# jasonyaw/CDAE

Hardware: AMD Instinct MI355X
Metric: users/sec (whole node) K=200 ML-10M-shape; Recall@10 parity (higher is better)
Workload: dtype f32

## Files before the change

cdae_amd/binding.py:

```python
from __future__ import annotations

import contextlib
import ctypes as C
import os
from dataclasses import dataclass

import numpy as np

_HERE = os.path.dirname(os.path.abspath(__file__))
LIB_PATH = os.environ.get("CDAE_HIP_LIBRARY") or os.path.join(_HERE, "lib", "libcdae_hip.so")
DEV_LIB_PATH = os.path.join(os.path.dirname(_HERE), "build", "libcdae_hip_dev.so")

SQUARE, LOGISTIC, LOG, HINGE, SQUARED_HINGE, CROSS_ENTROPY, LOGM = range(7)

P_W, P_W_AG, P_V, P_V_AG, P_WU, P_WU_AG, P_B, P_B_AG, P_BP, P_BP_AG, P_UU, P_UU_AG = range(12)
P_UB, P_UB_AG = 12, 13
P_COUNT = 14

PLAN_FUSED_DECODE, PLAN_GEMM2_TN, PLAN_ROWS_FUSED = 1, 2, 4
IMF_DEFAULT_BATCH_USERS = 16
BPR_DEFAULT_BATCH_USERS = 8
NO_USER = 0xFFFFFFFF
DEFAULT_BATCH_USERS = 0

# ... 14 lines not shown
    _fields_ = [("wall_seconds", C.c_double), ("users", C.c_uint64), ("examples", C.c_uint64),
                ("batches", C.c_uint64), ("ms_sample", C.c_double), ("ms_sort", C.c_double),
                ("ms_encode", C.c_double), ("ms_decode", C.c_double), ("ms_hidden", C.c_double),
                ("ms_input", C.c_double), ("launches_decode", C.c_uint64)]

    def as_dict(self):
        return {n: getattr(self, n) for n, _ in self._fields_}


EXPORTS = {
    "cdae_hip_last_error": (C.c_char_p, []),
    "cdae_hip_abi_version": (C.c_int, []),
    "cdae_hip_create": (C.c_int, [C.POINTER(_Config), C.c_int, C.POINTER(C.c_void_p)]),
    "cdae_hip_create_mf": (C.c_int, [C.POINTER(_MfConfig), C.c_int, C.POINTER(C.c_void_p)]),
    "cdae_hip_destroy": (C.c_int, [C.c_void_p]),
    "cdae_hip_set_interactions": (C.c_int, [C.c_void_p, C.c_uint64, C.c_uint64, C.c_void_p, C.c_void_p]),
    "cdae_hip_row_stride": (C.c_uint32, [C.c_void_p]),
    "cdae_hip_default_batch_users": (C.c_uint32, [C.c_uint64]),
    "cdae_hip_mf_default_batch_users": (C.c_uint32, [C.c_uint64, C.c_uint32]),
    "cdae_hip_batch_users": (C.c_uint32, [C.c_void_p]),
    "cdae_hip_full_output_plan": (C.c_uint32, [C.c_void_p]),
    "cdae_hip_set_decode_fused": (C.c_int, [C.c_void_p, C.c_int]),
    "cdae_hip_decode_plan": (C.c_int, [C.c_void_p, C.POINTER(C.c_uint32), C.POINTER(C.c_uint32), C.POINTER(C.c_uint32)]),
    "cdae_hip_user_order": (C.c_int, [C.c_void_p, C.c_void_p, C.c_size_t]),
    "cdae_hip_set_user_id_offset": (C.c_int, [C.c_void_p, C.c_uint64]),
    "cdae_hip_init_params": (C.c_int, [C.c_void_p, C.c_uint64]),
    "cdae_hip_set_param": (C.c_int, [C.c_void_p, C.c_uint32, C.c_void_p, C.c_size_t]),
    "cdae_hip_get_param": (C.c_int, [C.c_void_p, C.c_uint32, C.c_void_p, C.c_size_t]),
    "cdae_hip_param_device_ptr": (C.c_int, [C.c_void_p, C.c_uint32, C.POINTER(C.c_void_p), C.POINTER(C.c_size_t)]),
    "cdae_hip_train_epoch": (C.c_int, [C.c_void_p, C.c_uint64, C.c_uint32, C.POINTER(Stats)]),
    "cdae_hip_train_users": (C.c_int, [C.c_void_p, C.c_uint64, C.c_uint32, C.c_uint64, C.c_uint64, C.POINTER(Stats)]),
    "cdae_hip_enqueue_users": (C.c_int, [C.c_void_p, C.c_uint64, C.c_uint32, C.c_uint64, C.c_uint64]),
    "cdae_hip_prefetch_users": (C.c_int, [C.c_void_p, C.c_uint64, C.c_uint32, C.c_uint64, C.c_uint64]),
    "cdae_hip_collect_stats": (C.c_int, [C.c_void_p, C.POINTER(Stats)]),
    "cdae_hip_train_one_user_corruption": (C.c_int, [C.c_void_p, C.c_uint64, C.c_void_p, C.c_size_t, C.c_void_p, C.c_size_t]),
    "cdae_hip_set_profiling": (C.c_int, [C.c_void_p, C.c_int]),
    "cdae_hip_set_profiling_families": (C.c_int, [C.c_void_p, C.c_uint32]),
    "cdae_hip_synchronize": (C.c_int, [C.c_void_p]),
    "cdae_hip_debug_sample_batch": (C.c_int, [C.c_void_p, C.c_uint64, C.c_uint32, C.c_uint64, C.c_uint32, C.c_uint32] + [C.c_void_p] * 8
                                    + [C.POINTER(C.c_uint64)]),
    "cdae_hip_encode": (C.c_int, [C.c_void_p, C.c_uint64, C.c_uint32, C.c_int, C.c_void_p, C.c_size_t, C.c_void_p]),
    "cdae_hip_data_loss": (C.c_int, [C.c_void_p, C.c_uint64, C.c_uint32, C.POINTER(C.c_double)]),
    "cdae_hip_penalty_loss": (C.c_int, [C.c_void_p, C.POINTER(C.c_double)]),
    "cdae_hip_recommend_all": (C.c_int, [C.c_void_p, C.c_uint64, C.c_uint64, C.c_uint32, C.c_void_p]),
    "cdae_hip_recommend_user": (C.c_int, [C.c_void_p, C.c_uint64, C.c_void_p, C.c_size_t, C.c_uint32, C.c_void_p]),
    "cdae_hip_recommend_rows": (C.c_int, [C.c_void_p, C.c_uint64, C.c_void_p, C.c_void_p, C.c_void_p, C.c_uint32, C.c_void_p, C.c_void_p]),
# ... 141 lines not shown
    def reset(self, train, seed: int = 0):
        self.set_interactions(train.num_users, train.num_items, train.train_ptr, train.train_col)
        self.init_params(seed)

    def init_params(self, seed: int):
        _chk(self.lib, self.lib.cdae_hip_init_params(self.h, seed))

    def user_order(self) -> np.ndarray:
        out = np.empty(self.num_users, dtype=np.uint32)
        _chk(self.lib, self.lib.cdae_hip_user_order(self.h, out.ctypes.data, out.size))
        return out

    @property
    def batch_users(self) -> int:
        return int(self.lib.cdae_hip_batch_users(self.h))

    def set_decode_fused(self, allow: bool):
        _chk(self.lib, self.lib.cdae_hip_set_decode_fused(self.h, int(bool(allow))))

    @property
    def decode_plan(self) -> dict:
        a, b, c = C.c_uint32(0), C.c_uint32(0), C.c_uint32(0)
        _chk(self.lib, self.lib.cdae_hip_decode_plan(self.h, C.byref(a), C.byref(b), C.byref(c)))
        return dict(hot_rows=int(a.value), late_rows=int(b.value), fused=bool(c.value))

    @property
    def full_output_plan(self) -> int:
        return int(self.lib.cdae_hip_full_output_plan(self.h))

    def _shape(self, which):
        K = self.cfg.num_dim
        if which in (P_BP, P_BP_AG):
            return (self.num_items,)
        if which in (P_B, P_B_AG):
            return (K,)
        if which in (P_WU, P_WU_AG, P_UU, P_UU_AG):
            return (self.num_users, K)
        return (self.num_items, K)

    def get(self, which) -> np.ndarray:
        out = np.empty(self._shape(which), dtype=np.float32)
        _chk(self.lib, self.lib.cdae_hip_get_param(self.h, which, out.ctypes.data, out.size))
        return out

    def set(self, which, arr):
        a = np.ascontiguousarray(arr, dtype=np.float32).reshape(self._shape(which))
        _chk(self.lib, self.lib.cdae_hip_set_param(self.h, which, a.ctypes.data, a.size))
# ... 361 lines not shown
```

cdae_amd/csrc/cdae_hip.hip:

```cpp
#include <hip/hip_runtime.h>

#include <cstring>

#include <rocprim/rocprim.hpp>

#include <algorithm>
#include <atomic>
#include <condition_variable>
#include <deque>
#include <mutex>
#include <thread>
#include <chrono>
#include <cmath>
#include <cstdarg>
#include <cstdlib>
#include <cstdio>
#include <cstring>
#include <numeric>
#include <string>
#include <vector>

#include "../../include/cdae_hip.h"
#include "cdae_internal.hpp"
#include "cdae_kernels.hpp"
// ... 60 lines not shown
  uint64_t U = 0, I = 0;
  uint32_t K = 0, Kp = 0, NI = 1, B = 0;
  uint64_t uid_offset = 0;
  cdae::HyperParams hp{};

  std::vector<int64_t> h_row_ptr;
  int64_t* d_row_ptr = nullptr;
  uint32_t* d_col = nullptr;
  uint32_t* d_item_order = nullptr;
  uint32_t hot_rows = 0;
  uint32_t late_rows = 0;
  float* d_Ghot = nullptr;
  uint32_t* d_hotdup = nullptr;
  uint32_t* d_late_bits = nullptr;
  uint32_t late_words = 0;
  bool fused_decode = false;
  bool fused_possible = false;
  bool allow_fused = true;
  uint32_t* h_err = nullptr;
  int err_slot = -1;
  uint32_t* d_fused_err = nullptr;
  cdae::FusedGeom fused_geo{};
  bool fused_geo_set = false;
  std::vector<float> h_rank_len;
  uint32_t* d_cold_map = nullptr;
  uint32_t num_cus = 256;
  cdae::DecodeLate decode_late() const { return cdae::DecodeLate{d_Ghot, d_hotdup, late_rows}; }
  cdae::LateFinish late_finish() { return cdae::LateFinish{d_Ghot, d_hotdup, d_item_order, d_D0, d_dup_corr, late_rows}; }
  bool full_unfused = false;
  std::vector<uint32_t> h_unit_ptr;
  uint32_t* d_rank_of = nullptr;
  uint32_t* d_unit_user = nullptr;
  uint32_t* d_unit_ptr = nullptr;
  uint32_t unit_cap = 0;
  float* d_Hpart = nullptr;
  uint32_t* d_uptr_tmp = nullptr;

  float* d_shared = nullptr;
  size_t n_shared = 0, n_matrix = 0;
  size_t off[CDAE_P_COUNT] = {0};
  size_t cnt[CDAE_P_COUNT] = {0};
  float* d_Wu = nullptr;
  float* d_Wu_ag = nullptr;
  float* d_Uu = nullptr;
  float* d_Uu_ag = nullptr;
  float* d_Ssum = nullptr;
// ... 394 lines not shown
    HIPCHK(rocprim::radix_sort_pairs(sort_tmp, h->sort_tmp_bytes, x.key16, x.sorted_key16, x.val, x.sorted_val,
                                     (size_t)bt.E, 0u, (unsigned)h->sort_bits, st));
    hipLaunchKernelGGL(segment_kernel<uint16_t>, seg_grid, dim3(256), 0, st, x.sorted_key16, x.sorted_val, (uint32_t)bt.E,
                       x.seg, x.seg + I, x.dup_count, h->dup_cap, x.dup_of_pos, x.dup_of_ex, h->dup_stripes,
                       (const uint32_t*)h->d_rank_of, x.seg + 2 * (size_t)I, x.seg + 3 * (size_t)I, shs ? I : 0xFFFFFFFFu);
  } else {
    HIPCHK(rocprim::radix_sort_pairs(sort_tmp, h->sort_tmp_bytes, x.item, x.sorted_item, x.val, x.sorted_val,
                                     (size_t)bt.E, 0u, (unsigned)h->sort_bits, st));
    hipLaunchKernelGGL(segment_kernel<uint32_t>, seg_grid, dim3(256), 0, st, x.sorted_item, x.sorted_val, (uint32_t)bt.E,
                       x.seg, x.seg + I, x.dup_count, h->dup_cap, x.dup_of_pos, x.dup_of_ex, h->dup_stripes,
                       (const uint32_t*)h->d_rank_of, x.seg + 2 * (size_t)I, x.seg + 3 * (size_t)I, shs ? I : 0xFFFFFFFFu);
  }
  CHK(pr.end());
  if (h->cfg.full_output && h->d_bits_train) {
    const uint32_t words = (I + 31) / 32;
    uint32_t* bits = h->d_bits_train + (size_t)b * h->bits_stride;
    hipLaunchKernelGGL(rated_bits_kernel, dim3((bt.nb + 3) / 4), dim3(256), 0, st, h->d_row_ptr, h->d_col, bt.s0, bt.nb, words, bits);
  }
  HIPCHK(hipEventRecord(x.ready, st));
  HIPCHK(hipGetLastError());
  return 0;
}

int fused_geometry(cdae_hip* h, uint32_t hot, uint32_t I) {
  using namespace cdae;
  FusedGeom g{};
  g.hot_wgs = (hot + 3) / 4;
  const uint32_t n_groups = (I - hot + 3) / 4, S = h->num_cus;
  std::vector<float> len(n_groups, 0.f);
  for (uint32_t q = 0; q < n_groups; ++q)
    for (uint32_t j = 0; j < 4 && hot + 4 * q + j < I; ++j) len[q] = std::max(len[q], h->h_rank_len[hot + 4 * q + j]);
  std::vector<uint32_t> by_len(n_groups);
  std::iota(by_len.begin(), by_len.end(), 0u);
  std::stable_sort(by_len.begin(), by_len.end(), [&](uint32_t a, uint32_t b2) { return len[a] > len[b2]; });
  const uint32_t cu0 = std::min(g.hot_wgs, S > 8 ? S - 8 : 0u);
  const uint32_t n_bins = (S - cu0) * 4;
  std::vector<std::vector<uint32_t>> bin(n_bins);
  {
    using Ent = std::pair<float, uint32_t>;
    std::vector<Ent> heap;
    for (uint32_t i = 0; i < n_bins; ++i) heap.push_back({0.f, i});
    auto cmp = [](const Ent& a, const Ent& b2) { return a.first > b2.first || (a.first == b2.first && a.second > b2.second); };
    std::make_heap(heap.begin(), heap.end(), cmp);
    for (uint32_t k = 0; k < n_groups; ++k) {
      const uint32_t q = by_len[k];
      std::pop_heap(heap.begin(), heap.end(), cmp);
      Ent e = heap.back();
      bin[e.second].push_back(q);
      e.first += 4.f + len[q];
      heap.back() = e;
      std::push_heap(heap.begin(), heap.end(), cmp);
    }
  }
  size_t rounds_cold = 0;
  for (auto& v : bin) rounds_cold = std::max(rounds_cold, v.size());
  g.decode_wgs = (uint32_t)std::max<size_t>(rounds_cold, 1) * S;
  std::vector<uint32_t> map((size_t)g.decode_wgs * 4, 0xFFFFFFFFu);
  for (uint32_t i = 0; i < n_bins; ++i) {
    const uint32_t cu = cu0 + i / 4, w = i % 4;
    for (size_t k = 0; k < bin[i].size(); ++k) map[((size_t)k * S + cu) * 4 + w] = bin[i][k];
  }
  if (h->d_cold_map) { HIPCHK(hipFree(h->d_cold_map)); h->d_cold_map = nullptr; }
  CHK(dev_alloc(&h->d_cold_map, map.size()));
  HIPCHK(hipMemcpy(h->d_cold_map, map.data(), map.size() * sizeof(uint32_t), hipMemcpyHostToDevice));
  g.cold_map = h->d_cold_map;
  h->fused_geo = g;
  h->fused_geo_set = true;
  return 0;
}

int launch_decode(cdae_hip* h, cdae_hip::ExBuf& x, const cdae::GatherArgs* fused = nullptr) {
  using namespace cdae;
  hipStream_t st = h->stream;
  const uint32_t I = (uint32_t)h->I;
  const dim3 blk(256);
  const dim3 grid_rows((I + 3) / 4);
#define DECODE_TAIL h->d_item_order, x.seg + 2 * (size_t)I, x.seg + 3 * (size_t)I, x.sorted_val, h->d_Z, h->dec(), h->dec_ag(), \
                    h->P(CDAE_P_BP), h->P(CDAE_P_BP_AG), h->d_HG, h->d_G, h->d_D0, h->d_touched, x.dup_of_pos, h->d_dup_corr
#define DECODE_ARGS h->hp, DECODE_TAIL
#define DECODE_LA(NI_, L_, A_)                                                                                       \
  do {                                                                                                               \
    if (pad) hipLaunchKernelGGL((decode_rows_kernel<NI_, L_, A_, true>), grid_rows, blk, 0, st, DECODE_ARGS);        \
    else hipLaunchKernelGGL((decode_rows_kernel<NI_, L_, A_, false>), grid_rows, blk, 0, st, DECODE_ARGS);           \
  } while (0)
#define DECODE_NI(NI_)                                          \
  do {                                                          \
    if (ce && ada) DECODE_LA(NI_, 5, true);                     \
    else if (ce) DECODE_LA(NI_, 5, false);                      \
// ... 5 lines not shown
    if (fused) {                                                                                                       \
      if (ce && ada) hipLaunchKernelGGL((decode_gather_kernel<NV_, NT_, 5, true>), grid_fu, blk, 0, st, h->hp, hot, geo, late, *fused, DECODE_TAIL);   \
      else if (ce) hipLaunchKernelGGL((decode_gather_kernel<NV_, NT_, 5, false>), grid_fu, blk, 0, st, h->hp, hot, geo, late, *fused, DECODE_TAIL);    \
      else if (ada) hipLaunchKernelGGL((decode_gather_kernel<NV_, NT_, 0, true>), grid_fu, blk, 0, st, h->hp, hot, geo, late, *fused, DECODE_TAIL);    \
      else hipLaunchKernelGGL((decode_gather_kernel<NV_, NT_, 0, false>), grid_fu, blk, 0, st, h->hp, hot, geo, late, *fused, DECODE_TAIL);            \
    }                                                                                                                  \
    else if (ce && ada) hipLaunchKernelGGL((decode_hybrid_kernel<NV_, NT_, 5, true>), grid_hy, blk, 0, st, h->hp, hot, late, DECODE_TAIL);   \
    else if (ce) hipLaunchKernelGGL((decode_hybrid_kernel<NV_, NT_, 5, false>), grid_hy, blk, 0, st, h->hp, hot, late, DECODE_TAIL);    \
    else if (ada) hipLaunchKernelGGL((decode_hybrid_kernel<NV_, NT_, 0, true>), grid_hy, blk, 0, st, h->hp, hot, late, DECODE_TAIL);    \
    else hipLaunchKernelGGL((decode_hybrid_kernel<NV_, NT_, 0, false>), grid_hy, blk, 0, st, h->hp, hot, late, DECODE_TAIL);            \
  } while (0)
#define DECODE_HY_NT(NV_)                                                                        \
  do {                                                                                           \
    if (nt == 1) DECODE_HY(NV_, 1); else if (nt == 2) DECODE_HY(NV_, 2); else DECODE_HY(NV_, 4); \
  } while (0)
  {
    const bool ce = h->cfg.loss_type == CDAE_LOSS_CROSS_ENTROPY, ada = h->cfg.using_adagrad != 0, pad = h->K < h->Kp;
    const uint32_t K = h->K;
    if (K <= 256) {
      const uint32_t hot = std::min<uint32_t>(h->hot_rows, I);
      const uint32_t waves = hot + (I - hot + 3) / 4;
      const dim3 grid_hy((waves + 3) / 4);
      const DecodeLate late = h->decode_late();
      if (fused && !h->fused_geo_set) CHK(fused_geometry(h, hot, I));
      const FusedGeom geo = h->fused_geo;
      const dim3 grid_fu(geo.decode_wgs + (fused ? 8u * ((fused->n_units + 3u) / 4u) : 0u));
      const uint32_t nv = K / 64, tail = K % 64;
      const uint32_t nt = tail == 0 ? 0u : (tail < 16 ? 1u : (tail < 32 ? 2u : 4u));
      if (nt == 0) {
        switch (nv) { case 1: DECODE_HY(1, 0); break; case 2: DECODE_HY(2, 0); break; case 3: DECODE_HY(3, 0); break; default: DECODE_HY(4, 0); break; }
      } else {
        switch (nv) { case 0: DECODE_HY_NT(0); break; case 1: DECODE_HY_NT(1); break; case 2: DECODE_HY_NT(2); break; default: DECODE_HY_NT(3); break; }
      }
    } else {
      switch (h->NI) { case 1: DECODE_NI(1); break; case 2: DECODE_NI(2); break; case 4: DECODE_NI(4); break; default: DECODE_NI(8); break; }
    }
  }
#undef DECODE_HY_NT
#undef DECODE_HY
#undef DECODE_LA
#undef DECODE_NI
#undef DECODE_ARGS
#undef DECODE_TAIL
  HIPCHK(hipGetLastError());
  return 0;
}

// ... 566 lines not shown
}
int cdae_hip_user_order(cdae_hip_t* h, uint32_t* out, size_t count) {
  if (!h || !h->d_shared || !out) return fail("set_interactions must be called first");
  if (count != h->U) return fail("user order has %llu entries, got %zu", (unsigned long long)h->U, count);
  for (uint64_t pos = 0; pos < h->U; ++pos) out[pos] = h->user_perm.empty() ? (uint32_t)pos : h->user_perm[pos];
  return 0;
}
int cdae_hip_set_decode_fused(cdae_hip_t* h, int allow) {
  if (!h) return fail("null handle");
  h->allow_fused = allow != 0;
  h->fused_decode = h->fused_possible && h->allow_fused;
  return 0;
}

int cdae_hip_decode_plan(const cdae_hip_t* h, uint32_t* hot_rows, uint32_t* late_rows, uint32_t* fused) {
  if (!h) return fail("null handle");
  const bool set = h->d_shared != nullptr;
  if (hot_rows) *hot_rows = set && h->K <= 256 && !h->mf && !h->cfg.full_output ? h->hot_rows : 0u;
  if (late_rows) *late_rows = set ? h->late_rows : 0u;
  if (fused) *fused = set && h->fused_decode ? 1u : 0u;
  return 0;
}

uint32_t cdae_hip_batch_users(const cdae_hip_t* h) { return !h || (h->cfg.batch_users == 0 && h->U == 0) ? 0 : (h->mf_seq ? 1u : h->B); }
uint32_t cdae_hip_full_output_plan(const cdae_hip_t* h) {
  if (!h || !h->cfg.full_output || h->U == 0) return 0;
  if (h->Kp <= 256 && !h->full_unfused) return CDAE_PLAN_FUSED_DECODE;
  return (gemm2_tn_path(h) ? CDAE_PLAN_GEMM2_TN : 0u) | (rows_fused_path(h) ? CDAE_PLAN_ROWS_FUSED : 0u);
}

int cdae_hip_set_user_id_offset(cdae_hip_t* h, uint64_t offset) {
  if (!h) return fail("null handle");
  h->uid_offset = offset; h->hp.uid_offset = offset;
  return 0;
}

int cdae_hip_set_interactions(cdae_hip_t* h, uint64_t U, uint64_t I, const int64_t* row_ptr, const uint32_t* col) {
  if (!h || !row_ptr || (!col && U && row_ptr[U])) return fail("null argument");
  if (h->shard_sampled() && (!h->g_row_ptr_src || !h->g_col_src)) return fail("an item shard of the sampled decode needs the whole rows (set_item_shard_global)");
  if (h->shard_sampled() && h->mf) return fail("the item-sharded layout is CDAE's");
  if (U == 0 || I == 0) return fail("empty interaction matrix (%llu users, %llu items)", (unsigned long long)U, (unsigned long long)I);
  if (I >= (1ull << 30) || U >= (1ull << 30)) return fail("at most 2^30 users and items");
  if (row_ptr[0] != 0) return fail("row_ptr[0] must be 0");
  HIPCHK(hipSetDevice(h->device));
  CHK(join_aux(h));
  std::vector<int64_t> perm_ptr;
// ... 50 lines not shown
    h->B = cdae_hip_default_batch_users(U);
  }
  h->U = U; h->I = I; h->hp.num_items = (uint32_t)I;
  if (h->item_shard) {
    if (h->own_u1 == ~0ull) { h->own_u0 = 0; h->own_u1 = U; }
    if (h->own_u0 > h->own_u1 || h->own_u1 > U) return fail("owned user range [%llu, %llu) outside the %llu users", (unsigned long long)h->own_u0, (unsigned long long)h->own_u1, (unsigned long long)U);
    h->hp.own_u0 = h->own_u0; h->hp.own_u1 = h->own_u1;
  }
  {
    const uint64_t Bu = std::min<uint64_t>(h->B, U);
    h->hp.unit_pos = Bu <= 1024 ? 64u : cdae::UNIT_POS_MAX;
  }
  h->h_row_ptr.assign(row_ptr, row_ptr + U + 1);
  const size_t nnz = (size_t)row_ptr[U];
  CHK(dev_alloc(&h->d_row_ptr, U + 1));
  CHK(dev_alloc(&h->d_col, nnz));
  HIPCHK(hipMemcpy(h->d_row_ptr, row_ptr, (U + 1) * sizeof(int64_t), hipMemcpyHostToDevice));
  HIPCHK(hipMemcpy(h->d_col, col, nnz * sizeof(uint32_t), hipMemcpyHostToDevice));
  std::vector<uint32_t> order(I);
  std::iota(order.begin(), order.end(), 0u);
  std::stable_sort(order.begin(), order.end(), [&](uint32_t a, uint32_t b) { return pop[a] > pop[b]; });
  CHK(dev_alloc(&h->d_item_order, (size_t)I));
  HIPCHK(hipMemcpy(h->d_item_order, order.data(), I * sizeof(uint32_t), hipMemcpyHostToDevice));
  {
    std::vector<uint32_t> rank_of(I);
    for (uint32_t r = 0; r < I; ++r) rank_of[order[r]] = r;
    CHK(dev_alloc(&h->d_rank_of, (size_t)I));
    HIPCHK(hipMemcpy(h->d_rank_of, rank_of.data(), I * sizeof(uint32_t), hipMemcpyHostToDevice));
  }
  {
    const char* ev = DEV_ENV("CDAE_DECODE_HOT_POS");
    const double hot_pos = ev ? std::atof(ev) : 48.0;
    const double share = (double)std::min<uint64_t>(h->B, U) / (double)U;
    uint32_t hot = 0;
    while (hot < I && (double)pop[order[hot]] * share >= hot_pos) ++hot;
    h->hot_rows = std::min<uint32_t>((hot + 3u) & ~3u, (uint32_t)I);
  }
  {
    const bool hybrid = h->K <= 256 && !h->mf && !h->cfg.full_output;
    h->late_rows = 0;
    if (hybrid && I <= 32u * cdae::LATE_BITS_WORDS && !DEV_ENV("CDAE_NO_LATE_ROWS")) {
      const char* ev = DEV_ENV("CDAE_DECODE_LATE_POS");
      const double late_pos = ev ? std::atof(ev) : 48.0;
      const double share = (double)std::min<uint64_t>(h->B, U) / (double)U;
      uint32_t late = 0;
      while (late < I && late < cdae::LATE_MAX && (double)pop[order[late]] * share >= late_pos) ++late;
// ... 1625 lines not shown
```

cdae_amd/csrc/cdae_kernels.hpp:

```cpp
#pragma once
#include <type_traits>

#include <hip/hip_runtime.h>
#include <stdint.h>

#include "../../include/cdae_rng.h"
#include "cdae_exchange_algebra.h"

namespace cdae {

constexpr int WAVE = 64;
constexpr uint32_t SLOT_MASK = 0x0FFFFFFFu;
constexpr uint32_t DUP_PREV_BIT = 1u << 28;
constexpr uint32_t DUP_NEXT_BIT = 1u << 29;
constexpr uint32_t DUP_NONE = 0xFFFFFFFFu;
constexpr uint32_t DUP_STRIPES = 64;
constexpr uint32_t TARGET_BIT = 1u << 30;
constexpr uint32_t INPUT_BIT = 1u << 31;

constexpr uint32_t LATE_MAX = 64;
struct DecodeLate {
  float* Ghot;
  uint32_t* hotdup;
  uint32_t late_rows;
};
struct LateFinish {
  const float* Ghot; const uint32_t* hotdup; const uint32_t* items ; const float* D0; const float* dup_corr;
  uint32_t late_rows;
};
constexpr uint32_t G_PENDING = 0x7FC0DEADu;
// ... 1029 lines not shown
  }
#pragma unroll
  for (int i = 0; i < NT; ++i) base[64 * NV + l + 16 * i] = r[4 * NV + i];
}

template <int NV, int NT>
__device__ __forceinline__ void row16_store_sc1(float* __restrict__ matrix, uint32_t row_elem, const float (&r)[4 * NV + NT], uint32_t l) {
  const cdae_rsrc rs = rows_rsrc(matrix);
#pragma unroll
  for (int v = 0; v < NV; ++v) {
    cdae_b128 q; const float t[4] = {r[4 * v], r[4 * v + 1], r[4 * v + 2], r[4 * v + 3]};
    __builtin_memcpy(&q, t, sizeof q);
    __builtin_amdgcn_raw_buffer_store_b128(q, rs, (int)((row_elem + 64u * v + 4u * l) * 4u), 0, AUX_SC1);
  }
#pragma unroll
  for (int i = 0; i < NT; ++i)
    __builtin_amdgcn_raw_buffer_store_b32(__builtin_bit_cast(unsigned int, r[4 * NV + i]), rs, (int)((row_elem + 64u * NV + l + 16u * i) * 4u), 0, AUX_SC1);
}

constexpr uint32_t ROWS16_LDS_WORDS = 4u * 128u + 4u * 128u + 4u * 64u;
constexpr uint32_t ROW64_PARK_WORDS = ROWS16_LDS_WORDS;

template <int NV, int NT, int LOSS, bool ADAGRAD, bool FUSED = false>
__device__ __forceinline__ void decode_rows16(HyperParams hp, const uint32_t rank0, uint32_t* __restrict__ lds, CDAE_DECODE_PARAMS) {
  constexpr int GRP = 16, NE = 4 * NV + NT;
  constexpr bool HAS_PAD = NT > 0;
  const uint32_t lane = threadIdx.x % WAVE, l = lane & (GRP - 1), sub = lane / GRP;
  const uint32_t rank = rank0 + sub;
  const bool row_ok = rank < hp.num_items;
  const uint32_t item = row_ok ? item_order[rank] : 0u;
  const uint32_t beg = row_ok ? seg_begin[rank] : 0u, end = row_ok ? seg_end[rank] : 0u;
  const uint32_t n = end - beg;
  const uint32_t nmax = max(max((uint32_t)__builtin_amdgcn_readlane((int)n, 0), (uint32_t)__builtin_amdgcn_readlane((int)n, 16)),
                            max((uint32_t)__builtin_amdgcn_readlane((int)n, 32), (uint32_t)__builtin_amdgcn_readlane((int)n, 48)));
  if (nmax == 0) return;
  hp.loss_type = LOSS;
  hp.adagrad = ADAGRAD;
#ifdef CDAE_DECODE_TIMING
  unsigned long long* dbg = reinterpret_cast<unsigned long long*>(touched);
  int dbg_n = 0;
#define CDAE_STAMP() do { if (rank0 == hp.debug_rank && lane == 0 && dbg_n < 60) dbg[dbg_n++] = __builtin_readcyclecounter(); } while (0)
#else
#define CDAE_STAMP() do {} while (0)
#endif
  CDAE_STAMP();
  const bool tied = !hp.asymmetric;
  const bool pad_lane = HAS_PAD && l == GRP - 1;
  const float pad_one = pad_lane ? 1.f : 0.f;

  float w[NE], a[NE], wref[NE];
  const size_t row_off = (size_t)item * hp.Kp;
  if (n) {
    row16_load<NV, NT>(w, D + row_off, l);
// ... 242 lines not shown
      const uint32_t v = c + (uint32_t)h2 * WAVE + lane;
      const uint32_t e = example_of(v);
      const bool in = v < c_end;
      m.item[h2] = in ? ga.ex_item[base + e] : 0xFFFFFFFFu;
      if constexpr (FUSED) m.g[h2] = in ? load_f32_sc1(ga.G + base + e) : 0.f;
      else m.g[h2] = in ? ga.G[base + e] : 0.f;
      m.di[h2] = in ? ga.dup_of_ex[base + e] : DUP_NONE;
    }
  };
  auto is_mine = [&](uint32_t item) -> bool {
    bool mine = item < hp.num_items && (item & 7u) == part;
    if (lbits && mine) mine = ((lbits[item >> 5] >> (item & 31u)) & 1u) == 0u;
    return mine;
  };
  uint32_t head = 0, len = 0;
  auto trip = [&](uint32_t n_rows) {
    float vv[TRIP][NI], gg[TRIP];
#pragma unroll
    for (int t = 0; t < TRIP; ++t) {
      if ((uint32_t)t < n_rows) {
        const uint32_t e = (uint32_t)__builtin_amdgcn_readfirstlane((int)lrow[head + t]);
        gg[t] = __builtin_bit_cast(float, __builtin_amdgcn_readfirstlane(__builtin_bit_cast(int, lg[head + t])));
        if constexpr (FUSED) {
          vload_sc1<NI>(vv[t], (e & DUP_ROW) ? dc_rs : d0_rs, ((e & ~DUP_ROW) * hp.Kp + lo_ld) * 4u);
        } else {
          const float* src = (e & DUP_ROW) ? ga.dup_corr : ga.D0;
          vload<NI>(vv[t], src + (size_t)(e & ~DUP_ROW) * hp.Kp + lo_ld);
        }
      } else {
        gg[t] = 0.f;
#pragma unroll
        for (int k = 0; k < NI; ++k) vv[t][k] = 0.f;
      }
    }
#pragma unroll
    for (int t = 0; t < TRIP; ++t)
#pragma unroll
      for (int k = 0; k < NI; ++k) acc[k] = fmaf(gg[t], vv[t][k], acc[k]);
    head += n_rows;
  };
  Meta cur, nxt;
  load_meta(0u, n_ex, cur);
  for (uint32_t c0 = 0; c0 < n_ex; c0 += 2 * WAVE) {
    load_meta(c0 + 2 * WAVE, n_ex, nxt);
    if constexpr (FUSED) {
      for (uint32_t spin = 0;; ++spin) {
        const bool pend0 = __builtin_bit_cast(uint32_t, cur.g[0]) == G_PENDING && is_mine(cur.item[0]);
// ... 42 lines not shown
                     uint32_t n_units, uint64_t u0, uint32_t nb, const uint32_t* __restrict__ ex_item,
                     const float* __restrict__ G, const float* __restrict__ D0,
                     float* __restrict__ HGpart ,
                     uint32_t explicit_examples ,
                     const uint32_t* __restrict__ dup_of_ex, const float* __restrict__ dup_corr,
                     const uint32_t* __restrict__ unit_user,
                     const uint32_t* __restrict__ late_bits = nullptr ,
                     uint32_t late_words = 0) {
  __shared__ uint32_t gl_row[4][GATHER_CAP];
  __shared__ float gl_g[4][GATHER_CAP];
  __shared__ uint32_t lbits[LATE_BITS_WORDS];
  stage_late_bits(lbits, late_bits, late_words);
  const uint32_t part = blockIdx.x & 7u;
  const uint32_t unit = (blockIdx.x >> 3) * (blockDim.x / WAVE) + threadIdx.x / WAVE;
  if (unit >= n_units) return;
  const GatherArgs ga{row_ptr, uptr, n_units, u0, nb, ex_item, G, D0, HGpart, explicit_examples, dup_of_ex, dup_corr, unit_user,
                      late_bits, late_words, nullptr};
  hidden_gather_role<NI, false>(hp, ga, part, unit, gl_row[threadIdx.x / WAVE], gl_g[threadIdx.x / WAVE], late_bits ? lbits : nullptr);
}

struct FusedGeom {
  uint32_t hot_wgs;
  uint32_t decode_wgs;
  const uint32_t* cold_map;
};
constexpr uint32_t FUSED_LDS_WORDS = 4u * 2u * GATHER_CAP + LATE_BITS_WORDS;
static_assert(4u * ROWS16_LDS_WORDS <= FUSED_LDS_WORDS, "row roles' LDS");
static_assert(3u * (FUSED_LDS_WORDS + 8u) * 4u + 90376u <= 160u * 1024u, "three workgroups of this launch + one of bucket_sort_kernel per CU");
#ifndef CDAE_FUSED_WAVES_PER_SIMD
#define CDAE_FUSED_WAVES_PER_SIMD 3
#endif
template <int NV, int NT, int LOSS, bool ADAGRAD>
__global__ void __launch_bounds__(256, CDAE_FUSED_WAVES_PER_SIMD)
decode_gather_kernel(HyperParams hp, uint32_t hot_rows, FusedGeom geo, DecodeLate late, GatherArgs ga, CDAE_DECODE_PARAMS) {
  constexpr int CH = NT == 0 ? NV : NV + 1;
  constexpr int NI = CH <= 1 ? 1 : (CH <= 2 ? 2 : 4);
  __shared__ uint32_t fused_lds[FUSED_LDS_WORDS + 8u];
  const uint32_t wg = blockIdx.x;
  const uint32_t wid = __builtin_amdgcn_readfirstlane(threadIdx.x / WAVE);
  if (wg < geo.hot_wgs) {
    const uint32_t row = wg * 4u + wid;
    if (row < hot_rows && !CDAE_SKIP_ROLE(hp, 4u)) {
      const unsigned long long t0 = trace_begin(hp);
      __builtin_amdgcn_s_setprio(CDAE_HOT_PRIO);
      decode_row64<NI, LOSS, ADAGRAD, false, true>(hp, row, reinterpret_cast<float*>(fused_lds + wid * ROWS16_LDS_WORDS), ROW64_PARK_WORDS, late,
                                                   CDAE_DECODE_PASS);
      __builtin_amdgcn_s_setprio(0);
      trace_end(hp, 3, row, t0, hp.trace ? hw_place() : 0u);
    }
  } else if (wg < geo.decode_wgs) {
    if (CDAE_SKIP_ROLE(hp, 8u)) return;
    uint32_t* const claim = fused_lds + FUSED_LDS_WORDS;
    if (threadIdx.x < 4) claim[threadIdx.x] = 0u;
    __syncthreads();
    const uint32_t simd = (__builtin_amdgcn_s_getreg((1 << 11) | (4 << 6) | 4) ) & 3u;
    if (threadIdx.x % WAVE == 0) atomicCAS(&claim[simd], 0u, 1u + wid);
    __syncthreads();
    const uint32_t cs[4] = {claim[0], claim[1], claim[2], claim[3]};
    int mine = -1;
#pragma unroll
    for (int q = 0; q < 4; ++q) if (cs[q] == 1u + wid) mine = q;
    if (mine < 0) {
      uint32_t before = 0, cnt = 0;
#pragma unroll
      for (int q = 0; q < 4; ++q) if (cs[q] && cs[q] - 1u < wid) ++before;
      const uint32_t j = wid - before;
#pragma unroll
      for (int q = 0; q < 4; ++q) if (!cs[q]) { if (cnt == j) mine = q; ++cnt; }
    }
    const uint32_t g = geo.cold_map[wg * 4u + (uint32_t)mine];
    if (g == 0xFFFFFFFFu) return;
    const unsigned long long t0 = trace_begin(hp);
    decode_rows16<NV, NT, LOSS, ADAGRAD, true>(hp, hot_rows + g * 4u, fused_lds + wid * ROWS16_LDS_WORDS, CDAE_DECODE_PASS);
    trace_end(hp, 4, hot_rows / 4u + g, t0, hp.trace ? hw_place() : 0u);
  } else {
    uint32_t* const lbits = fused_lds + 4u * 2u * GATHER_CAP;
    stage_late_bits(lbits, ga.late_bits, ga.late_words);
    const uint32_t gw = wg - geo.decode_wgs;
    const uint32_t part = gw & 7u, unit = (gw >> 3) * 4u + wid;
    if (unit >= ga.n_units) return;
    hidden_gather_role<NI, true>(hp, ga, part, unit, fused_lds + wid * 2u * GATHER_CAP,
                                 reinterpret_cast<float*>(fused_lds + wid * 2u * GATHER_CAP + GATHER_CAP), ga.late_bits ? lbits : nullptr);
  }
}

template <int NI>
__device__ __forceinline__ void add_partial_rows(float (&hg)[NI], const float* __restrict__ HGpart, uint32_t n_units, uint32_t n_parts,
                                                 uint32_t ub, uint32_t ue, uint32_t Kp, uint32_t lo) {
  if (n_parts == 8u) {
    const size_t slab = (size_t)n_units * Kp;
    for (uint32_t u = ub; u < ue; u += 2) {
      const bool two = u + 1u < ue;
      const float* p0 = HGpart + (size_t)u * Kp + lo;
      const float* p1 = HGpart + (size_t)(two ? u + 1u : u) * Kp + lo;
      float a0[8][NI], a1[8][NI];
#pragma unroll
      for (int x = 0; x < 8; ++x) vload<NI>(a0[x], p0 + x * slab);
// ... 702 lines not shown
```

include/cdae_hip.h:

```cpp
#ifndef CDAE_HIP_H_
#define CDAE_HIP_H_

#include <stddef.h>
#include <stdint.h>

#ifdef __cplusplus
extern "C" {
#endif

#define CDAE_HIP_ABI_VERSION 12

#define CDAE_LOSS_SQUARE 0u
#define CDAE_LOSS_CROSS_ENTROPY 5u

#define CDAE_P_W 0u
#define CDAE_P_W_AG 1u
#define CDAE_P_V 2u
#define CDAE_P_V_AG 3u
#define CDAE_P_WU 4u
#define CDAE_P_WU_AG 5u
#define CDAE_P_B 6u
#define CDAE_P_B_AG 7u
#define CDAE_P_BP 8u
#define CDAE_P_BP_AG 9u
// ... 31 lines not shown
  uint64_t batches;
  double ms_sample, ms_sort, ms_encode, ms_decode, ms_hidden, ms_input;
  uint64_t launches_decode;
} cdae_hip_stats;

typedef struct cdae_hip cdae_hip_t;

const char* cdae_hip_last_error(void);
int cdae_hip_abi_version(void);

int cdae_hip_create(const cdae_hip_config* cfg, int device_id, cdae_hip_t** out);
int cdae_hip_destroy(cdae_hip_t* h);

int cdae_hip_set_interactions(cdae_hip_t* h, uint64_t num_users, uint64_t num_items,
                              const int64_t* row_ptr, const uint32_t* col_idx);

uint32_t cdae_hip_row_stride(const cdae_hip_t* h);

#define CDAE_DEFAULT_BATCH_USERS_MAX 256u
uint32_t cdae_hip_default_batch_users(uint64_t num_users);
uint32_t cdae_hip_batch_users(const cdae_hip_t* h);

int cdae_hip_decode_plan(const cdae_hip_t* h, uint32_t* hot_rows, uint32_t* late_rows, uint32_t* fused);
int cdae_hip_set_decode_fused(cdae_hip_t* h, int allow);

#define CDAE_PLAN_FUSED_DECODE 1u
#define CDAE_PLAN_GEMM2_TN 2u
#define CDAE_PLAN_ROWS_FUSED 4u
uint32_t cdae_hip_full_output_plan(const cdae_hip_t* h);

int cdae_hip_set_user_id_offset(cdae_hip_t* h, uint64_t global_id_of_local_user_0);

int cdae_hip_init_params(cdae_hip_t* h, uint64_t seed);

int cdae_hip_set_param(cdae_hip_t* h, uint32_t which, const float* host, size_t count);
int cdae_hip_get_param(cdae_hip_t* h, uint32_t which, float* host, size_t count);
int cdae_hip_param_device_ptr(cdae_hip_t* h, uint32_t which, void** device_ptr, size_t* padded_count);

int cdae_hip_train_epoch(cdae_hip_t* h, uint64_t seed, uint32_t epoch, cdae_hip_stats* stats);
int cdae_hip_train_users(cdae_hip_t* h, uint64_t seed, uint32_t epoch, uint64_t u_begin,
                         uint64_t u_end, cdae_hip_stats* stats);
int cdae_hip_enqueue_users(cdae_hip_t* h, uint64_t seed, uint32_t epoch, uint64_t u_begin, uint64_t u_end);
int cdae_hip_prefetch_users(cdae_hip_t* h, uint64_t seed, uint32_t epoch, uint64_t u_begin, uint64_t u_end);
int cdae_hip_collect_stats(cdae_hip_t* h, cdae_hip_stats* stats);

int cdae_hip_train_one_user_corruption(cdae_hip_t* h, uint64_t uid, const uint32_t* input_items,
// ... 123 lines not shown
```

Measured before the change: 2.908 million.

## Place fused decode row groups on XCDs matching item affinity

Replaces the fused decode cold-row map with a planner that groups cold item rows by item id modulo 8, so each group is scheduled on CUs of the XCD believed to own that item's data. It then load-balances across XCDs within a tolerance, and also remaps hot rows to affine workgroups. The kernel reads a precomputed (rank, item) pair per row instead of looking up item_order. Non-dup D0 rows are now loaded with a plain load instead of an sc1 load. The aim is better L2 locality on MI355X's multi-XCD layout, at the cost of less even grouping by length (lower fill) and a more complex plan.

```diff
diff --git a/cdae_amd/binding.py b/cdae_amd/binding.py
--- a/cdae_amd/binding.py
+++ b/cdae_amd/binding.py
@@ -60,6 +60,7 @@
     "cdae_hip_full_output_plan": (C.c_uint32, [C.c_void_p]),
     "cdae_hip_set_decode_fused": (C.c_int, [C.c_void_p, C.c_int]),
     "cdae_hip_decode_plan": (C.c_int, [C.c_void_p, C.POINTER(C.c_uint32), C.POINTER(C.c_uint32), C.POINTER(C.c_uint32)]),
+    "cdae_hip_decode_placement": (C.c_int, [C.c_void_p, C.POINTER(C.c_uint32), C.POINTER(C.c_uint32), C.POINTER(C.c_float), C.POINTER(C.c_float)]),
     "cdae_hip_user_order": (C.c_int, [C.c_void_p, C.c_void_p, C.c_size_t]),
     "cdae_hip_set_user_id_offset": (C.c_int, [C.c_void_p, C.c_uint64]),
     "cdae_hip_init_params": (C.c_int, [C.c_void_p, C.c_uint64]),
@@ -247,7 +248,10 @@
     def decode_plan(self) -> dict:
         a, b, c = C.c_uint32(0), C.c_uint32(0), C.c_uint32(0)
         _chk(self.lib, self.lib.cdae_hip_decode_plan(self.h, C.byref(a), C.byref(b), C.byref(c)))
-        return dict(hot_rows=int(a.value), late_rows=int(b.value), fused=bool(c.value))
+        p, q, fill, share = C.c_uint32(0), C.c_uint32(0), C.c_float(0), (C.c_float * 8)()
+        _chk(self.lib, self.lib.cdae_hip_decode_placement(self.h, C.byref(p), C.byref(q), C.byref(fill), share))
+        return dict(hot_rows=int(a.value), late_rows=int(b.value), fused=bool(c.value), placed_rows=int(p.value), affine_rows=int(q.value),
+                    group_fill=round(float(fill.value), 4), xcd_share=[round(float(x), 4) for x in share])
 
     @property
     def full_output_plan(self) -> int:
diff --git a/cdae_amd/csrc/cdae_fused_plan.hpp b/cdae_amd/csrc/cdae_fused_plan.hpp
--- /dev/null
+++ b/cdae_amd/csrc/cdae_fused_plan.hpp
@@ -0,0 +1,168 @@
+#pragma once
+#include <algorithm>
+#include <cstdint>
+#include <numeric>
+#include <utility>
+#include <vector>
+
+namespace cdae {
+
+constexpr uint32_t PLACED_NONE = 0xFFFFFFFFu;
+constexpr uint32_t PLACED_FOREIGN = 0x80000000u;
+constexpr float XCD_TOL = 0.03f;
+
+struct FusedPlan {
+  uint32_t hot_wgs = 0;
+  uint32_t decode_wgs = 0;
+  bool affine = false;
+  std::vector<uint32_t> hot_map;
+  std::vector<uint32_t> rows;
+  uint32_t placed_rows = 0;
+  uint32_t affine_rows = 0;
+  uint32_t groups = 0, foreign_groups = 0;
+  float fill = 0.f;
+  float xcd_share[8] = {0, 0, 0, 0, 0, 0, 0, 0};
+};
+
+inline FusedPlan build_fused_plan(const std::vector<uint32_t>& order, const std::vector<float>& rank_len, uint32_t hot, uint32_t late,
+                                  uint32_t S, bool want_affine = true) {
+  const uint32_t I = (uint32_t)order.size();
+  hot = std::min(hot, I);
+  late = std::min(late, hot);
+  FusedPlan p;
+  p.hot_wgs = (hot + 3) / 4;
+  p.affine = want_affine && S % 8 == 0 && S >= 16;
+  const uint32_t cu0 = std::min(p.hot_wgs, S > 8 ? S - 8 : 0u);
+  struct Group { uint32_t rank[4]; uint32_t n; float len; uint32_t res; uint32_t xcd; };
+  std::vector<Group> gr;
+  auto close_group = [&](Group& g) {
+    g.len = 0.f;
+    for (uint32_t j = 0; j < g.n; ++j) g.len = std::max(g.len, rank_len[g.rank[j]]);
+    gr.push_back(g);
+    g.n = 0;
+  };
+  if (p.affine) {
+    Group open[8];
+    for (uint32_t r = 0; r < 8; ++r) { open[r].n = 0; open[r].res = r; open[r].xcd = r; }
+    for (uint32_t rank = hot; rank < I; ++rank) {
+      Group& g = open[order[rank] & 7u];
+      g.rank[g.n++] = rank;
+      if (g.n == 4) close_group(g);
+    }
+    for (uint32_t r = 0; r < 8; ++r) if (open[r].n) close_group(open[r]);
+  } else {
+    Group g; g.n = 0; g.res = 0; g.xcd = 0;
+    for (uint32_t rank = hot; rank < I; ++rank) {
+      g.rank[g.n++] = rank;
+      if (g.n == 4) close_group(g);
+    }
+    if (g.n) close_group(g);
+  }
+  const uint32_t n_groups = (uint32_t)gr.size();
+  p.groups = n_groups;
+  auto cost = [&](uint32_t q) { return 4.f + gr[q].len; };
+  std::vector<uint32_t> by_len(n_groups);
+  std::iota(by_len.begin(), by_len.end(), 0u);
+  std::stable_sort(by_len.begin(), by_len.end(), [&](uint32_t a, uint32_t b) { return gr[a].len > gr[b].len; });
+  const uint32_t n_bins = (S - cu0) * 4;
+  const uint32_t n_pools = p.affine ? 8u : 1u;
+  std::vector<std::vector<uint32_t>> pool_groups(n_pools);
+  float bins_of[8] = {0, 0, 0, 0, 0, 0, 0, 0}, load[8] = {0, 0, 0, 0, 0, 0, 0, 0};
+  if (p.affine) {
+    for (uint32_t cu = cu0; cu < S; ++cu) bins_of[cu & 7u] += 4.f;
+    float total = 0.f, max_cost = 0.f;
+    for (uint32_t q = 0; q < n_groups; ++q) { total += cost(q); max_cost = std::max(max_cost, cost(q)); }
+    auto share = [&](uint32_t x) { return total * bins_of[x] / (float)n_bins; };
+    auto rel = [&](uint32_t x) { return load[x] / bins_of[x]; };
+    for (uint32_t k = 0; k < n_groups; ++k) {
+      const uint32_t q = by_len[k];
+      uint32_t x = gr[q].res;
+      if (load[x] + cost(q) > share(x) * (1.f + XCD_TOL) + max_cost) {
+        for (uint32_t y = 0; y < 8; ++y) if (rel(y) < rel(x)) x = y;
+      }
+      gr[q].xcd = x;
+      load[x] += cost(q);
+      pool_groups[x].push_back(q);
+    }
+    for (uint32_t it = 0; it < n_groups; ++it) {
+      uint32_t lo = 0, hi = 0;
+      for (uint32_t y = 1; y < 8; ++y) { if (rel(y) < rel(lo)) lo = y; if (rel(y) > rel(hi)) hi = y; }
+      if (load[lo] >= share(lo) * (1.f - XCD_TOL) - max_cost || lo == hi || pool_groups[hi].empty()) break;
+      const uint32_t q = pool_groups[hi].back();
+      if ((load[hi] - cost(q)) / bins_of[hi] < (load[lo] + cost(q)) / bins_of[lo]) break;
+      pool_groups[hi].pop_back();
+      load[hi] -= cost(q);
+      gr[q].xcd = lo;
+      load[lo] += cost(q);
+      pool_groups[lo].push_back(q);
+    }
+    for (uint32_t x = 0; x < 8; ++x) {
+      std::stable_sort(pool_groups[x].begin(), pool_groups[x].end(), [&](uint32_t a, uint32_t b) { return gr[a].len > gr[b].len; });
+      p.xcd_share[x] = total > 0.f ? load[x] / share(x) : 1.f;
+    }
+  } else {
+    pool_groups[0] = by_len;
+  }
+  std::vector<std::vector<uint32_t>> bin(n_bins);
+  for (uint32_t x = 0; x < n_pools; ++x) {
+    using Ent = std::pair<float, uint32_t>;
+    std::vector<Ent> heap;
+    for (uint32_t i = 0; i < n_bins; ++i)
+      if (!p.affine || ((cu0 + i / 4) & 7u) == x) heap.push_back({0.f, i});
+    auto cmp = [](const Ent& a, const Ent& b) { return a.first > b.first || (a.first == b.first && a.second > b.second); };
+    std::make_heap(heap.begin(), heap.end(), cmp);
+    for (uint32_t q : pool_groups[x]) {
+      std::pop_heap(heap.begin(), heap.end(), cmp);
+      Ent e = heap.back();
+      bin[e.second].push_back(q);
+      e.first += cost(q);
+      heap.back() = e;
+      std::push_heap(heap.begin(), heap.end(), cmp);
+    }
+  }
+  size_t rounds = 0;
+  for (auto& v : bin) rounds = std::max(rounds, v.size());
+  p.decode_wgs = (uint32_t)std::max<size_t>(rounds, 1) * S;
+  p.rows.assign((size_t)p.decode_wgs * 32, 0u);
+  for (size_t i = 0; i < p.rows.size(); i += 2) p.rows[i] = PLACED_NONE;
+  double ex = 0., slots = 0.;
+  for (uint32_t i = 0; i < n_bins; ++i) {
+    const uint32_t cu = cu0 + i / 4, w = i % 4;
+    for (size_t k = 0; k < bin[i].size(); ++k) {
+      const Group& g = gr[bin[i][k]];
+      const bool foreign = p.affine && g.xcd != g.res;
+      uint32_t* e = &p.rows[(((size_t)k * S + cu) * 4 + w) * 8];
+      for (uint32_t j = 0; j < g.n; ++j) {
+        e[2 * j] = g.rank[j] | (foreign || !p.affine ? PLACED_FOREIGN : 0u);
+        e[2 * j + 1] = order[g.rank[j]];
+        ex += rank_len[g.rank[j]];
+      }
+      slots += 4. * g.len;
+      p.placed_rows += g.n;
+      if (p.affine && !foreign) p.affine_rows += g.n;
+      if (foreign) ++p.foreign_groups;
+    }
+  }
+  p.fill = slots > 0. ? (float)(ex / slots) : 1.f;
+  p.placed_rows += hot - late;
+  if (p.affine && hot > late) {
+    p.hot_map.assign((size_t)p.hot_wgs * 4, PLACED_NONE);
+    std::vector<uint32_t> rest;
+    for (uint32_t rank = 0; rank < late; ++rank) rest.push_back(rank | PLACED_FOREIGN);
+    for (uint32_t rank = late; rank < hot; ++rank) {
+      bool done = false;
+      for (uint32_t wg = order[rank] & 7u; wg < p.hot_wgs && !done; wg += 8)
+        for (uint32_t w = 0; w < 4 && !done; ++w)
+          if (p.hot_map[wg * 4 + w] == PLACED_NONE) { p.hot_map[wg * 4 + w] = rank; done = true; }
+      if (done) ++p.affine_rows; else rest.push_back(rank | PLACED_FOREIGN);
+    }
+    size_t s = 0;
+    for (uint32_t e : rest) {
+      while (p.hot_map[s] != PLACED_NONE) ++s;
+      p.hot_map[s] = e;
+    }
+  }
+  return p;
+}
+
+}
diff --git a/cdae_amd/csrc/cdae_hip.hip b/cdae_amd/csrc/cdae_hip.hip
--- a/cdae_amd/csrc/cdae_hip.hip
+++ b/cdae_amd/csrc/cdae_hip.hip
@@ -106,6 +106,7 @@
   uint32_t* d_fused_err = nullptr;
   cdae::FusedGeom fused_geo{};
   bool fused_geo_set = false;
+  std::vector<uint32_t> h_order;
   std::vector<float> h_rank_len;
   uint32_t* d_cold_map = nullptr;
   uint32_t num_cus = 256;
@@ -546,48 +547,23 @@
   return 0;
 }
 
-int fused_geometry(cdae_hip* h, uint32_t hot, uint32_t I) {
+cdae::FusedPlan fused_plan(const cdae_hip* h) {
+  const uint32_t hot = std::min<uint32_t>(h->hot_rows, (uint32_t)h->I);
+  return cdae::build_fused_plan(h->h_order, h->h_rank_len, hot, h->late_rows, h->num_cus, !DEV_ENV("CDAE_FUSED_NO_AFFINITY"));
+}
+int fused_geometry(cdae_hip* h) {
   using namespace cdae;
+  const FusedPlan p = fused_plan(h);
   FusedGeom g{};
-  g.hot_wgs = (hot + 3) / 4;
-  const uint32_t n_groups = (I - hot + 3) / 4, S = h->num_cus;
-  std::vector<float> len(n_groups, 0.f);
-  for (uint32_t q = 0; q < n_groups; ++q)
-    for (uint32_t j = 0; j < 4 && hot + 4 * q + j < I; ++j) len[q] = std::max(len[q], h->h_rank_len[hot + 4 * q + j]);
-  std::vector<uint32_t> by_len(n_groups);
-  std::iota(by_len.begin(), by_len.end(), 0u);
-  std::stable_sort(by_len.begin(), by_len.end(), [&](uint32_t a, uint32_t b2) { return len[a] > len[b2]; });
-  const uint32_t cu0 = std::min(g.hot_wgs, S > 8 ? S - 8 : 0u);
-  const uint32_t n_bins = (S - cu0) * 4;
-  std::vector<std::vector<uint32_t>> bin(n_bins);
-  {
-    using Ent = std::pair<float, uint32_t>;
-    std::vector<Ent> heap;
-    for (uint32_t i = 0; i < n_bins; ++i) heap.push_back({0.f, i});
-    auto cmp = [](const Ent& a, const Ent& b2) { return a.first > b2.first || (a.first == b2.first && a.second > b2.second); };
-    std::make_heap(heap.begin(), heap.end(), cmp);
-    for (uint32_t k = 0; k < n_groups; ++k) {
-      const uint32_t q = by_len[k];
-      std::pop_heap(heap.begin(), heap.end(), cmp);
-      Ent e = heap.back();
-      bin[e.second].push_back(q);
-      e.first += 4.f + len[q];
-      heap.back() = e;
-      std::push_heap(heap.begin(), heap.end(), cmp);
-    }
-  }
-  size_t rounds_cold = 0;
-  for (auto& v : bin) rounds_cold = std::max(rounds_cold, v.size());
-  g.decode_wgs = (uint32_t)std::max<size_t>(rounds_cold, 1) * S;
-  std::vector<uint32_t> map((size_t)g.decode_wgs * 4, 0xFFFFFFFFu);
-  for (uint32_t i = 0; i < n_bins; ++i) {
-    const uint32_t cu = cu0 + i / 4, w = i % 4;
-    for (size_t k = 0; k < bin[i].size(); ++k) map[((size_t)k * S + cu) * 4 + w] = bin[i][k];
-  }
+  g.hot_wgs = p.hot_wgs;
+  g.decode_wgs = p.decode_wgs;
   if (h->d_cold_map) { HIPCHK(hipFree(h->d_cold_map)); h->d_cold_map = nullptr; }
-  CHK(dev_alloc(&h->d_cold_map, map.size()));
-  HIPCHK(hipMemcpy(h->d_cold_map, map.data(), map.size() * sizeof(uint32_t), hipMemcpyHostToDevice));
-  g.cold_map = h->d_cold_map;
+  CHK(dev_alloc(&h->d_cold_map, p.rows.size() + p.hot_map.size()));
+  HIPCHK(hipMemcpy(h->d_cold_map, p.rows.data(), p.rows.size() * sizeof(uint32_t), hipMemcpyHostToDevice));
+  if (!p.hot_map.empty())
+    HIPCHK(hipMemcpy(h->d_cold_map + p.rows.size(), p.hot_map.data(), p.hot_map.size() * sizeof(uint32_t), hipMemcpyHostToDevice));
+  g.rows = reinterpret_cast<const uint2*>(h->d_cold_map);
+  g.hot_map = p.hot_map.empty() ? nullptr : h->d_cold_map + p.rows.size();
   h->fused_geo = g;
   h->fused_geo_set = true;
   return 0;
@@ -639,7 +615,7 @@
       const uint32_t waves = hot + (I - hot + 3) / 4;
       const dim3 grid_hy((waves + 3) / 4);
       const DecodeLate late = h->decode_late();
-      if (fused && !h->fused_geo_set) CHK(fused_geometry(h, hot, I));
+      if (fused && !h->fused_geo_set) CHK(fused_geometry(h));
       const FusedGeom geo = h->fused_geo;
       const dim3 grid_fu(geo.decode_wgs + (fused ? 8u * ((fused->n_units + 3u) / 4u) : 0u));
       const uint32_t nv = K / 64, tail = K % 64;
@@ -1252,6 +1228,18 @@
   return 0;
 }
 
+int cdae_hip_decode_placement(const cdae_hip_t* h, uint32_t* placed_rows, uint32_t* affine_rows, float* group_fill, float* xcd_share) {
+  if (!h) return fail("null handle");
+  const bool set = h->d_shared != nullptr && h->fused_possible;
+  cdae::FusedPlan p;
+  if (set) p = fused_plan(h);
+  if (placed_rows) *placed_rows = p.placed_rows;
+  if (affine_rows) *affine_rows = p.affine_rows;
+  if (group_fill) *group_fill = p.fill;
+  if (xcd_share) for (int x = 0; x < 8; ++x) xcd_share[x] = p.xcd_share[x];
+  return 0;
+}
+
 uint32_t cdae_hip_batch_users(const cdae_hip_t* h) { return !h || (h->cfg.batch_users == 0 && h->U == 0) ? 0 : (h->mf_seq ? 1u : h->B); }
 uint32_t cdae_hip_full_output_plan(const cdae_hip_t* h) {
   if (!h || !h->cfg.full_output || h->U == 0) return 0;
@@ -1348,6 +1336,7 @@
   std::stable_sort(order.begin(), order.end(), [&](uint32_t a, uint32_t b) { return pop[a] > pop[b]; });
   CHK(dev_alloc(&h->d_item_order, (size_t)I));
   HIPCHK(hipMemcpy(h->d_item_order, order.data(), I * sizeof(uint32_t), hipMemcpyHostToDevice));
+  h->h_order = order;
   {
     std::vector<uint32_t> rank_of(I);
     for (uint32_t r = 0; r < I; ++r) rank_of[order[r]] = r;
diff --git a/cdae_amd/csrc/cdae_kernels.hpp b/cdae_amd/csrc/cdae_kernels.hpp
--- a/cdae_amd/csrc/cdae_kernels.hpp
+++ b/cdae_amd/csrc/cdae_kernels.hpp
@@ -6,6 +6,7 @@
 
 #include "../../include/cdae_rng.h"
 #include "cdae_exchange_algebra.h"
+#include "cdae_fused_plan.hpp"
 
 namespace cdae {
 
@@ -1081,13 +1082,19 @@
 constexpr uint32_t ROW64_PARK_WORDS = ROWS16_LDS_WORDS;
 
 template <int NV, int NT, int LOSS, bool ADAGRAD, bool FUSED = false>
-__device__ __forceinline__ void decode_rows16(HyperParams hp, const uint32_t rank0, uint32_t* __restrict__ lds, CDAE_DECODE_PARAMS) {
+__device__ __forceinline__ void decode_rows16(HyperParams hp, const uint32_t rank0, uint32_t* __restrict__ lds, CDAE_DECODE_PARAMS,
+                                              const uint2* __restrict__ placed = nullptr) {
   constexpr int GRP = 16, NE = 4 * NV + NT;
   constexpr bool HAS_PAD = NT > 0;
   const uint32_t lane = threadIdx.x % WAVE, l = lane & (GRP - 1), sub = lane / GRP;
-  const uint32_t rank = rank0 + sub;
+  uint32_t rank = rank0 + sub, item = 0u;
+  if constexpr (FUSED) {
+    const uint2 e = placed[sub];
+    rank = e.x == PLACED_NONE ? PLACED_NONE : e.x & ~PLACED_FOREIGN;
+    item = e.y;
+  }
   const bool row_ok = rank < hp.num_items;
-  const uint32_t item = row_ok ? item_order[rank] : 0u;
+  if constexpr (!FUSED) item = row_ok ? item_order[rank] : 0u;
   const uint32_t beg = row_ok ? seg_begin[rank] : 0u, end = row_ok ? seg_end[rank] : 0u;
   const uint32_t n = end - beg;
   const uint32_t nmax = max(max((uint32_t)__builtin_amdgcn_readlane((int)n, 0), (uint32_t)__builtin_amdgcn_readlane((int)n, 16)),
@@ -1376,7 +1383,8 @@
         const uint32_t e = (uint32_t)__builtin_amdgcn_readfirstlane((int)lrow[head + t]);
         gg[t] = __builtin_bit_cast(float, __builtin_amdgcn_readfirstlane(__builtin_bit_cast(int, lg[head + t])));
         if constexpr (FUSED) {
-          vload_sc1<NI>(vv[t], (e & DUP_ROW) ? dc_rs : d0_rs, ((e & ~DUP_ROW) * hp.Kp + lo_ld) * 4u);
+          if (e & DUP_ROW) vload_sc1<NI>(vv[t], dc_rs, ((e & ~DUP_ROW) * hp.Kp + lo_ld) * 4u);
+          else vload<NI>(vv[t], ga.D0 + (size_t)e * hp.Kp + lo_ld);
         } else {
           const float* src = (e & DUP_ROW) ? ga.dup_corr : ga.D0;
           vload<NI>(vv[t], src + (size_t)(e & ~DUP_ROW) * hp.Kp + lo_ld);
@@ -1465,7 +1473,8 @@
 struct FusedGeom {
   uint32_t hot_wgs;
   uint32_t decode_wgs;
-  const uint32_t* cold_map;
+  const uint2* rows;
+  const uint32_t* hot_map;
 };
 constexpr uint32_t FUSED_LDS_WORDS = 4u * 2u * GATHER_CAP + LATE_BITS_WORDS;
 static_assert(4u * ROWS16_LDS_WORDS <= FUSED_LDS_WORDS, "row roles' LDS");
@@ -1482,7 +1491,11 @@
   const uint32_t wg = blockIdx.x;
   const uint32_t wid = __builtin_amdgcn_readfirstlane(threadIdx.x / WAVE);
   if (wg < geo.hot_wgs) {
-    const uint32_t row = wg * 4u + wid;
+    uint32_t row = wg * 4u + wid;
+    if (geo.hot_map) {
+      const uint32_t e = geo.hot_map[row];
+      row = e == PLACED_NONE ? PLACED_NONE : e & ~PLACED_FOREIGN;
+    }
     if (row < hot_rows && !CDAE_SKIP_ROLE(hp, 4u)) {
       const unsigned long long t0 = trace_begin(hp);
       __builtin_amdgcn_s_setprio(CDAE_HOT_PRIO);
@@ -1511,11 +1524,12 @@
 #pragma unroll
       for (int q = 0; q < 4; ++q) if (!cs[q]) { if (cnt == j) mine = q; ++cnt; }
     }
-    const uint32_t g = geo.cold_map[wg * 4u + (uint32_t)mine];
-    if (g == 0xFFFFFFFFu) return;
+    const uint32_t slot = wg * 4u + (uint32_t)mine;
+    const uint2* const placed = geo.rows + slot * 4u;
+    if (placed[0].x == PLACED_NONE) return;
     const unsigned long long t0 = trace_begin(hp);
-    decode_rows16<NV, NT, LOSS, ADAGRAD, true>(hp, hot_rows + g * 4u, fused_lds + wid * ROWS16_LDS_WORDS, CDAE_DECODE_PASS);
-    trace_end(hp, 4, hot_rows / 4u + g, t0, hp.trace ? hw_place() : 0u);
+    decode_rows16<NV, NT, LOSS, ADAGRAD, true>(hp, 0u, fused_lds + wid * ROWS16_LDS_WORDS, CDAE_DECODE_PASS, placed);
+    trace_end(hp, 4, slot, t0, hp.trace ? hw_place() : 0u);
   } else {
     uint32_t* const lbits = fused_lds + 4u * 2u * GATHER_CAP;
     stage_late_bits(lbits, ga.late_bits, ga.late_words);
diff --git a/include/cdae_hip.h b/include/cdae_hip.h
--- a/include/cdae_hip.h
+++ b/include/cdae_hip.h
@@ -77,6 +77,7 @@
 uint32_t cdae_hip_batch_users(const cdae_hip_t* h);
 
 int cdae_hip_decode_plan(const cdae_hip_t* h, uint32_t* hot_rows, uint32_t* late_rows, uint32_t* fused);
+int cdae_hip_decode_placement(const cdae_hip_t* h, uint32_t* placed_rows, uint32_t* affine_rows, float* group_fill, float* xcd_share);
 int cdae_hip_set_decode_fused(cdae_hip_t* h, int allow);
 
 #define CDAE_PLAN_FUSED_DECODE 1u
```

After: 2.649 million. 0.911x the previous value.
